# Immortalqx/pi-slam-fusion

Measured on AMD Instinct MI355X. Metric: keyframes/sec fused (4000x3000 -> 256^2 tiles, 5-band), higher is better.
Workload: dtype f32; 1 GPU; cfg-2/cfg-A: 4000x3000 BGR8 keyframes, serpentine sortie, Map2D.Scale=1, 5-band Laplacian, CV_32FC3 (ForceFloat=1) pyramids, frames resident in HBM; frames_per_rank=2646, sortie_frames_before_timing=20, lookahead=48, rendered_rank0=2666, culled_tiles_rank0=490117

## Files before the change

include/pifusion.h:

```cpp
#ifndef PIFUSION_H
#define PIFUSION_H
#include <stddef.h>
#include <stdint.h>

#ifdef __cplusplus
extern "C" {
#endif

#define PF_ELE_PIXELS 256

enum { PF_TYPE_NONE = 0, PF_TYPE_CPU = 1, PF_TYPE_GPU = 2, PF_TYPE_MULTIBAND = 3, PF_TYPE_RENDER = 4 };

enum { PF_8UC1 = 0, PF_8UC3 = 16, PF_8UC4 = 24, PF_16SC3 = 19, PF_32FC1 = 5, PF_32FC3 = 21 };

typedef struct pf_image {
    int         rows, cols, type;
    const void* data;
    size_t      step;
} pf_image;

typedef struct pf_options {
    int    band_number;
    int    force_float;
    int    high_quality_show;
    int    weight_type;
    int    bg_color;
    double resolution;
    double scale;
    int    device;
    int    shard_rank;
    int    shard_count;
    int    shard_block;
    int    max_queue;
    int    fused;
    int    lookahead;
} pf_options;

typedef struct pf_map pf_map;

void    pf_default_options(pf_options* o);
int     pf_options_set(pf_options* o, const char* key, const char* value);
pf_map* pf_create(int type, int thread, const pf_options* opt);
void    pf_destroy(pf_map* m);
const char* pf_last_error(void);

int     pf_prepare(pf_map* m, const double plane[7], const double cam[6],
                   int n, const pf_image* imgs, const double* poses7);
int     pf_feed(pf_map* m, const pf_image* img, const double pose[7]);
int     pf_feed_device(pf_map* m, const pf_image* img, const double pose[7]);
long    pf_debug_read_last_frame(pf_map* m, void* out, size_t cap);
int     pf_debug_phase_stamps(unsigned long long* out, int cap_blocks);
int     pf_debug_select_counts(unsigned long long* out, int reset);
unsigned pf_queue_size(pf_map* m);
int     pf_sync(pf_map* m);
int     pf_save(pf_map* m, const char* filename);
int     pf_save_tiff(pf_map* m, const char* filename, int quality, int force_bigtiff);
int     pf_save_tiff_masked(pf_map* m, const char* filename, int quality, int force_bigtiff);
int     pf_write_image(const char* filename, const uint8_t* bgr, int rows, int cols);
int     pf_tiff_write_bgr(const char* filename, const uint8_t* bgr, int rows, int cols, size_t step, int quality, int bg,
                          const double model_transform[16], int force_bigtiff);
int     pf_tiff_write_device(const char* filename, const void* dev_bgr, int rows, int cols, size_t step, int quality, int bg,
                             const double model_transform[16], int force_bigtiff, void* hip_stream);
int     pf_tiff_write_bgr_masked(const char* filename, const uint8_t* bgr, int rows, int cols, size_t step,
                                 const uint8_t* mask, size_t mask_step, int quality, int bg,
                                 const double model_transform[16], int force_bigtiff);
int     pf_tiff_write_device_masked(const char* filename, const void* dev_bgr, int rows, int cols, size_t step,
                                    const void* dev_mask, size_t mask_step, int quality, int bg,
                                    const double model_transform[16], int force_bigtiff, void* hip_stream);
int     pf_jpeg_encode_bgr(const uint8_t* bgr, int rows, int cols, size_t step, int quality, uint8_t* out, size_t cap, size_t* len);
int     pf_jpeg_encode_device(const void* dev_bgr, int rows, int cols, size_t step, int quality, uint8_t* out, size_t cap, size_t* len, void* hip_stream);
int     pf_image_info(const char* filename, int* rows, int* cols);
int     pf_read_image(const char* filename, uint8_t* bgr, int rows, int cols);
int     pf_jpeg_info(const uint8_t* data, size_t len, int* rows, int* cols, int* components);
int     pf_jpeg_decode_bgr(const uint8_t* data, size_t len, uint8_t* bgr, int rows, int cols);
int     pf_jpeg_decode_device(const uint8_t* data, size_t len, void* dev_bgr, int rows, int cols, void* hip_stream);
void    pf_debug_jpeg_huffman(pf_map* m, long long out[3]);
int     pf_feed_jpeg(pf_map* m, const uint8_t* data, size_t len, const double pose[7]);
int     pf_feed_jpeg_batch(pf_map* m, int n, const uint8_t* const* data, const size_t* len, const double* poses7, int threads, int* results);
int     pf_save_to_memory(pf_map* m, uint8_t* bgr, int* rows, int* cols, int* tile_x0, int* tile_y0);
int     pf_save_to_memory_mask(pf_map* m, uint8_t* bgr, uint8_t* mask, int* rows, int* cols, int* tile_x0, int* tile_y0);

int     pf_num_levels(pf_map* m);
int     pf_pyramid_type(pf_map* m);
int     pf_grid(pf_map* m, int dims[4], double geo[6]);
int     pf_tile_count(pf_map* m);
int     pf_tile_coords(pf_map* m, int* xy, int cap);
int     pf_get_tile_level(pf_map* m, int ix, int iy, int level, void* lap, float* w);
int     pf_get_tile_bgra(pf_map* m, int ix, int iy, uint8_t* bgra256);
int     pf_blend_tile_raw(pf_map* m, int ix, int iy, void* out);
int     pf_blend_tile(pf_map* m, int ix, int iy, uint8_t* bgr256);
int     pf_blend_changed(pf_map* m, int* xy, uint8_t* bgr, int cap);
int     pf_blend_tiles(pf_map* m, const int* xy, int n, uint8_t* bgr);
int     pf_blend_tiles_jpeg(pf_map* m, const int* xy, int n, int quality, uint8_t* out, size_t cap, size_t* offsets);
int     pf_blend_tiles_level(pf_map* m, const int* xy, int n, int level, uint8_t* bgr, void* raw);
int     pf_blend_changed_level(pf_map* m, int level, int* xy, uint8_t* bgr, int cap);
int     pf_save_to_memory_level(pf_map* m, int level, uint8_t* bgr, int* rows, int* cols, int* tile_x0, int* tile_y0);
void*   pf_host_alloc(size_t bytes);
void    pf_host_free(void* p);
int     pf_format_map_update(const double plane[7], const double gps_origin[3], double min_x, double min_y, double ele_size,
                             int x, int y, char* out, int cap);
int     pf_map_update_command(pf_map* m, int ix, int iy, const double gps_origin[3], char* out, int cap);
void    pf_lnglat_from_distance(double lng1, double lat1, double dx, double dy, double* lng2, double* lat2);
int     pf_normalize_using_weight_map(const float* weight, float* src3, size_t npix);
int     pf_mul_weight_map(const float* weight, float* src3, size_t npix);

// ... 64 lines not shown
```

pi-slam-fusion_amd/csrc/c_api.cpp:

```cpp
#include "dist.hpp"
#include "jpeg_device.hpp"
#include <cstdlib>
#include <cmath>
#include <cstdio>
#include <cstring>
#include <algorithm>
#include <vector>
#include <mutex>
#include <new>

using pf::FusionMap;

struct pf_map {
    FusionMap impl;
    pf::JpegDevice jpeg;
    pf_map(int t, bool th, const pf_options& o) : impl(t, th, o) {}
    ~pf_map() { if (impl.ok() && impl.use_device()) impl.sync(); }
};

static std::mutex g_jpeg_mu;
static pf::JpegDevice* shared_jpeg(int device = 0)
{
    static pf::JpegDevice* d[64] = {};
    if (device < 0 || device >= 64) device = 0;
// ... 9 lines not shown
    o->resolution = 0; o->scale = 1; o->device = -1; o->shard_rank = 0; o->shard_count = 1; o->shard_block = 8;
    o->max_queue = 20; o->fused = 1; o->lookahead = 48;
}

int pf_options_set(pf_options* o, const char* key, const char* value)
{
    if (!o || !key || !value) return 0;
    const double v = std::atof(value);
    if (!std::strcmp(key, "MultiBandMap2DCPU.BandNumber")) o->band_number = (int)v;
    else if (!std::strcmp(key, "MultiBandMap2DCPU.ForceFloat")) o->force_float = (int)v;
    else if (!std::strcmp(key, "MultiBandMap2DCPU.HighQualityShow")) o->high_quality_show = (int)v;
    else if (!std::strcmp(key, "Map2D.WeightType")) o->weight_type = (int)v;
    else if (!std::strcmp(key, "Result.BackGroundColor")) o->bg_color = (int)v;
    else if (!std::strcmp(key, "Map2D.Resolution")) o->resolution = v;
    else if (!std::strcmp(key, "Map2D.Scale")) o->scale = v;
    else if (!std::strcmp(key, "Device")) o->device = (int)v;
    else if (!std::strcmp(key, "Shard.Rank")) o->shard_rank = (int)v;
    else if (!std::strcmp(key, "Shard.Count")) o->shard_count = (int)v;
    else if (!std::strcmp(key, "Shard.Block")) o->shard_block = (int)v;
    else if (!std::strcmp(key, "Map2D.MaxQueue")) o->max_queue = (int)v;
    else if (!std::strcmp(key, "Fused")) o->fused = (int)v;
    else if (!std::strcmp(key, "Lookahead")) o->lookahead = (int)v;
    else return 0;
    return 1;
}

pf_map* pf_create(int type, int thread, const pf_options* opt)
{
    if (type == PF_TYPE_NONE || type == PF_TYPE_RENDER) return nullptr;
    pf_options o;
    if (opt) o = *opt; else pf_default_options(&o);
    pf_map* m = new (std::nothrow) pf_map(type, thread != 0, o);
    if (m && !m->impl.ok()) { delete m; return nullptr; }
    return m;
}

void pf_destroy(pf_map* m) { delete m; }
const char* pf_last_error(void) { return pf::last_error(); }

int pf_prepare(pf_map* m, const double plane[7], const double cam[6], int n, const pf_image* imgs, const double* poses7)
{ return m && m->impl.prepare(plane, cam, n, imgs, poses7); }

int pf_feed(pf_map* m, const pf_image* img, const double pose[7]) { return m && m->impl.feed(img, pose, false); }
int pf_feed_device(pf_map* m, const pf_image* img, const double pose[7]) { return m && m->impl.feed(img, pose, true); }
int pf_debug_phase_stamps(unsigned long long* out, int cap_blocks) { return pf::read_phase_stamps(out, cap_blocks); }
void pf_debug_form_counts(long long out[8]) { if (out) pf::read_form_counts(out); }
long long pf_debug_compact_launches(void) { return pf::read_compact_launches(); }
int pf_debug_render_log(pf_map* m, long long* out, int cap) { return m ? m->impl.render_log(out, cap) : 0; }
void pf_set_cull(pf_map* m, int on) { if (m) m->impl.set_cull(on != 0); }
long long pf_debug_culled_cells(pf_map* m) { return m ? m->impl.culled_cells() : 0; }
double pf_debug_level0_exact_px(pf_map* m) { return m ? m->impl.level0_exact_px() : 0; }
long long pf_debug_culled_tiles(pf_map* m) { return m ? m->impl.culled_tiles() : 0; }
int pf_debug_select_counts(unsigned long long* out, int reset) { return out ? pf::read_select_counts(out, reset) : 0; }
long pf_debug_read_last_frame(pf_map* m, void* out, size_t cap) { return m ? m->impl.read_back_last_frame(out, cap) : -1; }
unsigned pf_queue_size(pf_map* m) { return m ? m->impl.queue_size() : 0; }
int pf_sync(pf_map* m) { return m && m->impl.sync(); }
int pf_save(pf_map* m, const char* filename) { return m && filename && m->impl.save(filename); }
int pf_save_tiff(pf_map* m, const char* filename, int quality, int force_bigtiff) { return m && filename && m->impl.save_tiff(filename, quality, force_bigtiff != 0); }
int pf_save_tiff_masked(pf_map* m, const char* filename, int quality, int force_bigtiff) { return m && filename && m->impl.save_tiff_masked(filename, quality, force_bigtiff != 0); }
int pf_jpeg_info(const uint8_t* data, size_t len, int* rows, int* cols, int* components) { return pf::jpeg_info(data, len, rows, cols, components); }
int pf_jpeg_decode_bgr(const uint8_t* data, size_t len, uint8_t* bgr, int rows, int cols)
{ return rows > 0 && cols > 0 && pf::jpeg_decode_bgr(data, len, bgr, rows, cols, (size_t)cols * 3); }
int pf_jpeg_decode_device(const uint8_t* data, size_t len, void* dev_bgr, int rows, int cols, void* hip_stream)
{
    std::lock_guard<std::mutex> l(g_jpeg_mu);
    if (rows <= 0 || cols <= 0 || !dev_bgr) return 0;
    hipPointerAttribute_t at{};
    if (hipPointerGetAttributes(&at, dev_bgr) != hipSuccess || at.type != hipMemoryTypeDevice) { (void)hipGetLastError(); pf::set_error("pf_jpeg_decode_device: destination is not device memory"); return 0; }
    int prev = 0;
    (void)hipGetDevice(&prev);
    if (at.device != prev && hipSetDevice(at.device) != hipSuccess) { pf::set_error("pf_jpeg_decode_device: hipSetDevice failed"); return 0; }
    const int ok = shared_jpeg(at.device)->decode_to(data, len, (uint8_t*)dev_bgr, rows, cols, hip_stream);
    if (at.device != prev) (void)hipSetDevice(prev);
    return ok;
}
static pf::JpegEncoder* shared_jpeg_encoder(int device)
{
    static pf::JpegEncoder* e[64] = {};
    if (device < 0 || device >= 64) device = 0;
    if (!e[device]) e[device] = new pf::JpegEncoder();
    return e[device];
}
int pf_jpeg_encode_device(const void* dev_bgr, int rows, int cols, size_t step, int quality, uint8_t* out, size_t cap, size_t* len, void* hip_stream)
{
    std::lock_guard<std::mutex> l(g_jpeg_mu);
    if (!dev_bgr || !len || rows <= 0 || cols <= 0) { pf::set_error("pf_jpeg_encode_device: no image, no length or a size that is not positive"); return 0; }
    if (!pf::jpeg_size_ok("pf_jpeg_encode_device", rows, cols)) return 0;
    if (step == 0) step = (size_t)cols * 3;
    if (step < (size_t)cols * 3) { pf::set_error("pf_jpeg_encode_device: step is smaller than a row"); return 0; }
    if (!out) { *len = pf::jenc::stream_bound(rows, cols); return 1; }
    hipPointerAttribute_t at{};
    if (hipPointerGetAttributes(&at, dev_bgr) != hipSuccess || at.type != hipMemoryTypeDevice) { (void)hipGetLastError(); pf::set_error("pf_jpeg_encode_device: the image is not in device memory"); return 0; }
    int prev = 0;
    (void)hipGetDevice(&prev);
    if (at.device != prev && hipSetDevice(at.device) != hipSuccess) { pf::set_error("pf_jpeg_encode_device: hipSetDevice failed"); return 0; }
    pf::JpegEncoder* e = shared_jpeg_encoder(at.device);
    size_t off[2] = { 0, 0 };
    int ok = e->encode(dev_bgr, 1, nullptr, 0, rows, cols, step, quality, off, hip_stream);
    if (ok) {
        *len = off[1];
        if (off[1] > cap) {
            pf::set_error("pf_jpeg_encode_device: the stream has " + std::to_string(off[1]) + " bytes, the buffer " + std::to_string(cap));
            (void)hipStreamSynchronize((hipStream_t)hip_stream);
            ok = 0;
        } else ok = e->fetch(out, hip_stream);
    }
// ... 308 lines not shown
```

pi-slam-fusion_amd/csrc/kernels.hip:

```cpp
#include "kernels.hpp"
#include "warp_index.hpp"
#include "env.hpp"
#include <climits>
#include <cmath>
#include <cstdlib>
#include <type_traits>

#ifndef PF_EXPERIMENTS
#define PF_EXPERIMENTS 0
#endif
#ifndef PF_ROWTAB
#define PF_ROWTAB 0
#endif
#ifndef PF_HYBRID_W
#define PF_HYBRID_W 0
#endif

namespace pf {

constexpr bool kExp = PF_EXPERIMENTS != 0;

__device__ __forceinline__ double clamp_int_range(double v)
{
    v = (v < (double)INT_MAX) ? v : (double)INT_MAX;
// ... 753 lines not shown
        }
        u.w = 0.f;
        U[p][lx] = u;
    }
    lds_barrier();
#pragma unroll
    for (int it = 0; it < ND; it++) {
        const uint64_t ent = ents[it];
        if (!ent) continue;
        const int idx = tid + it * LNT, ly = idx >> 6, lx = idx & 63;
        const int y = y0 + ly, x = x0 + lx;
        const Px gpx = A[ly + 4][lx + 4];
        if (!(gpx.w >= dwv[it])) continue;
        const uint64_t slot = ent & ~(uint64_t)1;
        const int loc = (y & (ts - 1)) * ts + (x & (ts - 1));
        const int sy = y >> 1;
        int syn = sy + 1; if (syn >= nrows) syn = nrows - 1;
        int syp = sy - 1; if (syp < 0) syp = nrows > 1 ? 1 : 0;
        const Hx u1 = U[sy - by0][lx], u2 = U[syn - by0][lx];
        T out[3];
        if (y & 1) {
#pragma unroll
            for (int k = 0; k < 3; k++) out[k] = sat_sub(gpx.c[k], cast_up((u1.c[k] + u2.c[k]) * 4));
        } else {
            const Hx u0 = U[syp - by0][lx];
#pragma unroll
            for (int k = 0; k < 3; k++) out[k] = sat_sub(gpx.c[k], cast_up(u0.c[k] + u1.c[k] * 6 + u2.c[k]));
        }
        T PF_GLOBAL* dl = (T PF_GLOBAL*)(slot + lay.lap_off) + loc * 3;
        dl[0] = out[0]; dl[1] = out[1]; dl[2] = out[2];
        ((float PF_GLOBAL*)(slot + lay.w_off))[loc] = gpx.w;
    }
    if (st + 1 < LS) {
        lds_barrier();
        Px keep;
        const bool mv = tid < 7 * LAW;
        if (mv) keep = (&A[0][0])[LBH * LAW + tid];
        lds_barrier();
        if (mv) (&A[0][0])[tid] = keep;
    }
    }
}

__device__ __forceinline__ void phase_stamp(unsigned long long* st, int slot)
{
    if (st) {
        unsigned long long t;
        asm volatile("s_memtime %0\n\ts_waitcnt lgkmcnt(0)" : "=s"(t) :: "memory");
        if (threadIdx.x == 0) st[slot] = t;
    }
}

__device__ unsigned long long g_select_seen[kMaxLevels], g_select_won[kMaxLevels];

constexpr int kPatchBytes = 81920 - 44928;

template <bool F32, int LBH, int LNT, bool STAMP = false, int ILP = 2, bool PATCH = false, bool WA = false, class LO = LevelOffsets, class GA = LevelArgs>
__device__ __forceinline__ void level3_block(const bool FROM_WARP, const LO& lay, const GA& g, const FusedWarp& wa,
                                             const uint8_t* __restrict__ src, const PxT<F32>* __restrict__ gw_in,
                                             PxT<F32>* __restrict__ gw_out, const uint64_t* __restrict__ table_generic, const int b,
                                             unsigned long long* stamps = nullptr, const uint64_t* tab0 = nullptr)
{
    const uint64_t PF_GLOBAL* __restrict__ table = (const uint64_t PF_GLOBAL*)table_generic;
    if (STAMP) phase_stamp(stamps, 0);
    struct StampExit { unsigned long long* st; __device__ StampExit(unsigned long long* p) : st(p) {} __device__ ~StampExit() { asm volatile("s_waitcnt vmcnt(0)" ::: "memory"); phase_stamp(st, 5); } };
    struct NoExit { __device__ NoExit(unsigned long long*) {} };
    typename std::conditional<STAMP, StampExit, NoExit>::type at_exit(stamps);
    (void)at_exit;
    using T = typename Pix<F32>::T; using WT = typename Pix<F32>::WT;
    using Px = PxT<F32>;
    constexpr int LAH = LBH + 7, LQH = LBH / 2 + 2;
    static_assert(LNT >= 32 * (LBH / 2), "one thread per 2x2 output quad (threads beyond that help in stages A and B only)");
    struct Bx { T c[F32 ? 3 : 4]; };
    constexpr int kPitch = LBH == 24 ? LAW : 2 * LAWH;
    __shared__ Px A[LAH][kPitch];
    constexpr int kTail = PATCH ? kPatchBytes : (int)(sizeof(Bx) * LQH * LQW);
    static_assert(kTail >= (int)(sizeof(Bx) * LQH * LQW), "Bt must fit");
    __shared__ __attribute__((aligned(16))) unsigned char tail[kTail];
    Bx (*Bt)[LQW] = reinterpret_cast<Bx (*)[LQW]>(tail);
    auto Aat = [&](int r, int c) -> Px& { return A[r][(c & 1) * LAWH + (c >> 1)]; };
    static_assert(LBH != 32 || PATCH || sizeof(A) + sizeof(tail) <= (F32 ? 42 : 32) * 1280, "LDS budget (64x32 blocks)");
    static_assert(LBH != 24 || sizeof(A) + sizeof(tail) <= 32 * 1280, "LDS budget (64x24 blocks: four workgroups per CU for both pyramid types)");
    static_assert(LBH != 32 || !PATCH || sizeof(A) + sizeof(tail) <= 64 * 1280, "LDS budget (64x32 blocks with a source patch: two per CU)");
    static_assert(LBH != 64 || sizeof(A) + sizeof(tail) <= (F32 ? 128 : 64) * 1280, "LDS budget (64x64 blocks of 1024 threads: int16 two per CU, fp32 one)");

    int bx, by; block_xy(g, b, bx, by);
    const int x0 = g.cx0 + bx * LBW, y0 = g.cy0 + by * LBH;
    const int ax0 = x0 - 4, ay0 = y0 - 4;
    const int nrows = g.rows >> 1, ncols = g.cols >> 1;
    const int bx0 = (x0 >> 1) - 1, by0 = (y0 >> 1) - 1;
    const int tid = threadIdx.x;
    const int sh = 8 - g.level, ts = kElePixels >> g.level;
    if (kExp && (g.ablate & 512) && !FROM_WARP) __builtin_amdgcn_s_setprio(2);

    const int qx = tid & 31, qy = tid >> 5;
    const int dx0 = x0 + 2 * qx, dy0 = y0 + 2 * qy;
    uint64_t ent = 0;
    if (tid < 32 * (LBH / 2) && dx0 < g.cols && dy0 < g.rows) {
        const int ti = (dy0 >> sh) * g.tiles_x + (dx0 >> sh);
        if (tab0) ent = ((const uint64_t PF_GLOBAL*)tab0)[ti];
        else ent = table[ti];
        if (sh >= 3) { if (cell_culled(ent, dx0, dy0, ts, sh)) ent = 0; }
        else {
            bool all = true;
#pragma unroll
            for (int k = 0; k < 4; k++) all = all && cell_culled(ent, dx0 + (k & 1), dy0 + (k >> 1), ts, sh);
            if (all) ent = 0;
        }
        ent &= ~kEntCells;
    }

    if (kExp && FROM_WARP && (g.ablate & 1024) && tid >= LNT / 2) __builtin_amdgcn_s_setprio(1);
    if (kExp && FROM_WARP && (g.ablate & 2048) && tid < LNT / 2) __builtin_amdgcn_s_setprio(1);
    if (FROM_WARP) {
        const bool inner = ax0 >= 0 && ax0 + LAW <= g.cols && ay0 >= 0 && ay0 + LAH <= g.rows;
        constexpr int RS = LNT / LAW;
        const int r0 = tid / LAW, c = tid - r0 * LAW;
        const bool near101 = g.rows >= 8 && g.cols >= 8;
        auto col_of = [&](int cc) {
            int x = ax0 + cc;
            if (!inner) x = near101 ? border_reflect101_near(x, g.cols) : border_reflect101(x, g.cols);
            return x;
        };
        auto row_of = [&](int r) {
            int y = ay0 + r;
            if (!inner) y = near101 ? border_reflect101_near(y, g.rows) : border_reflect101(y, g.rows);
            return y;
        };
// ... 317 lines not shown
            auto emit = [&](int e) {
                const int p = 2 * pp + e, Y = by0 + p;
                if (Y < 0 || Y >= nrows) return;
                Px o;
                {
                    const us2 v01 = h01[2 * e + 2] * (us2)6 + (h01[2 * e + 1] + h01[2 * e + 3]) * (us2)4 + h01[2 * e] + h01[2 * e + 4];
                    const us2 v2p = h2p[2 * e + 2] * (us2)6 + (h2p[2 * e + 1] + h2p[2 * e + 3]) * (us2)4 + h2p[2 * e] + h2p[2 * e + 4];
                    const us2 o01 = (v01 + (us2)128) >> (us2)8, o2p = (v2p + (us2)128) >> (us2)8;
                    o.c[0] = (short)o01.x; o.c[1] = (short)o01.y; o.c[2] = (short)o2p.x;
                }
                {
                    const float r0 = hw[2 * e], r1 = hw[2 * e + 1], r2 = hw[2 * e + 2], r3 = hw[2 * e + 3], r4 = hw[2 * e + 4];
                    if (X < vec_w) {
                        float a = r0 + r4;
                        const float bb = (r1 + r3) + r2;
                        a = a + (r2 + r2);
                        o.w = (a + bb * 4.f) * (1.f / 256);
                    } else
                        o.w = (r2 * 6 + (r1 + r3) * 4 + r0 + r4) * (1.f / 256);
                }
                o.pad = 0;
                {
                    Bx ob; ob.c[0] = o.c[0]; ob.c[1] = o.c[1]; ob.c[2] = o.c[2]; ob.c[3] = 0;
                    Bt[p][q] = ob;
                }
                if (p >= 1 && p < LQH - 1 && q >= 1 && q < LQW - 1) {
                    if (kExp && (g.ablate & 4096)) {
                        typedef uint32_t u2g __attribute__((ext_vector_type(2)));
                        u2g v; __builtin_memcpy(&v, &o, 8);
                        if (g.write_next) ((u2g*)gw_out)[(long)Y * ncols + X] = v;
                    } else
                    if (g.write_next) gw_out[(long)Y * ncols + X] = o;
                    if (g.top_select) select_store<F32>(lay.top_lap_off, lay.top_w_off, g.level + 1, table, g.tiles_x, X, Y, o.c, o.w);
                }
            };
#pragma unroll
            for (int j = 0; j < 7; j++) {
                const PxP* ev = reinterpret_cast<const PxP*>(&A[4 * pp + j][q]); const PxP* od = reinterpret_cast<const PxP*>(&A[4 * pp + j][LAWH + q]);
                const PxP a0 = ev[0], a1 = od[0], a2 = ev[1], a3 = od[1], a4 = ev[2];
                h01[j] = a2.c01 * (us2)6 + (a1.c01 + a3.c01) * (us2)4 + a0.c01 + a4.c01;
                h2p[j] = a2.c2p * (us2)6 + (a1.c2p + a3.c2p) * (us2)4 + a0.c2p + a4.c2p;
                hw[j] = a2.w * 6 + (a1.w + a3.w) * 4 + a0.w + a4.w;
                asm volatile("" : "+v"(h01[j]), "+v"(h2p[j]), "+v"(hw[j]) :: "memory");
                if (j == 4) emit(0);
                if (j == 6) emit(1);
            }
        }
    }
    if (STAMP) phase_stamp(stamps, 3);
    lds_barrier();
    if (STAMP) phase_stamp(stamps, 4);
    if (kExp && (g.ablate & 4)) return;

    if (!ent) return;
    int ry = dy0;
    asm volatile("" : "+v"(ry));
    ry -= y0;
    const Px g00 = A[ry + 4][qx + 2], g01 = A[ry + 4][LAWH + qx + 2];
    const Px g10 = A[ry + 5][qx + 2], g11 = A[ry + 5][LAWH + qx + 2];
    const bool in01 = dx0 + 1 < g.cols, in10 = dy0 + 1 < g.rows;
    const bool s00 = g00.w >= dwv[0][0], s01 = in01 && g01.w >= dwv[0][1];
    const bool s10 = in10 && g10.w >= dwv[1][0], s11 = in10 && in01 && g11.w >= dwv[1][1];
#ifdef PF_COUNT_WINS
    if constexpr (STAMP) {
        atomicAdd(&g_select_seen[g.level], (unsigned long long)(1 + (int)in01 + (int)in10 + (int)(in10 && in01)));
        atomicAdd(&g_select_won[g.level], (unsigned long long)((int)s00 + (int)s01 + (int)s10 + (int)s11));
    }
#endif
    if (!(s00 || s01 || s10 || s11)) return;
    const int sy = dy0 >> 1, sx = dx0 >> 1;
    int syn = sy + 1; if (syn >= nrows) syn = nrows - 1;
    int syp = sy - 1; if (syp < 0) syp = nrows > 1 ? 1 : 0;
    const bool one = ncols == 1, le = sx == 0, re = sx == ncols - 1;
    const bool edge = le || re;
    const int j = qx + 1;
    const int ja = (le && !F32) ? (one ? j : j + 1) : j - 1, jc = (re && !F32) ? j : j + 1;
    const int rows3[3] = { syp - by0, sy - by0, syn - by0 };
    T PF_GLOBAL* dl = (T PF_GLOBAL*)(slot + lay.lap_off) + loc0 * 3;
    float PF_GLOBAL* dw = (float PF_GLOBAL*)(slot + lay.w_off) + loc0;
    if constexpr (F32) {
        if (__builtin_amdgcn_ballot_w64(edge) == 0) {
            f2 heL[3], hoL[3]; float he2[3], ho2[3];
#pragma unroll
            for (int r = 0; r < 3; r++) {
                const float* pa = Bt[rows3[r]][j - 1].c; const float* pb = Bt[rows3[r]][j].c; const float* pc = Bt[rows3[r]][j + 1].c;
                const f2 aL = { pa[0], pa[1] }, bL = { pb[0], pb[1] }, cL = { pc[0], pc[1] };
                const float a2 = pa[2], b2 = pb[2], c2 = pc[2];
                heL[r] = aL + bL * 6.f + cL; hoL[r] = (bL + cL) * 4.f;
                he2[r] = a2 + b2 * 6 + c2;   ho2[r] = (b2 + c2) * 4;
            }
            const f2 g00L = { g00.c[0], g00.c[1] }, g01L = { g01.c[0], g01.c[1] }, g10L = { g10.c[0], g10.c[1] }, g11L = { g11.c[0], g11.c[1] };
            const f2 o00L = g00L - (heL[0] + heL[1] * 6.f + heL[2]) * (1.f / 64);
            const f2 o01L = g01L - (hoL[0] + hoL[1] * 6.f + hoL[2]) * (1.f / 64);
            const f2 o10L = g10L - ((heL[1] + heL[2]) * 4.f) * (1.f / 64);
            const f2 o11L = g11L - ((hoL[1] + hoL[2]) * 4.f) * (1.f / 64);
            const float o00c = g00.c[2] - (he2[0] + he2[1] * 6 + he2[2]) * (1.f / 64);
            const float o01c = g01.c[2] - (ho2[0] + ho2[1] * 6 + ho2[2]) * (1.f / 64);
            const float o10c = g10.c[2] - ((he2[1] + he2[2]) * 4) * (1.f / 64);
            const float o11c = g11.c[2] - ((ho2[1] + ho2[2]) * 4) * (1.f / 64);
            auto st3 = [&](T PF_GLOBAL* p, float a, float b, float c2) { PF_STORE(p, a); PF_STORE(p + 1, b); PF_STORE(p + 2, c2); };
            if (s00) { st3(dl, o00L.x, o00L.y, o00c); PF_STORE_W(&dw[0], g00.w); }
            if (s01) { st3(dl + 3, o01L.x, o01L.y, o01c); PF_STORE_W(&dw[1], g01.w); }
            if (s10) { st3(dl + 3 * ts, o10L.x, o10L.y, o10c); PF_STORE_W(&dw[ts], g10.w); }
            if (s11) { st3(dl + 3 * ts + 3, o11L.x, o11L.y, o11c); PF_STORE_W(&dw[ts + 1], g11.w); }
            return;
        }
    }
    if constexpr (!F32) {
        ss2 he01[3], ho01[3], he2p[3], ho2p[3];
#pragma unroll
        for (int r = 0; r < 3; r++) {
            const BxP a = *reinterpret_cast<const BxP*>(&Bt[rows3[r]][ja]), bq = *reinterpret_cast<const BxP*>(&Bt[rows3[r]][j]),
                      c = *reinterpret_cast<const BxP*>(&Bt[rows3[r]][jc]);
            he01[r] = a.c01 + bq.c01 * (ss2)6 + c.c01; ho01[r] = (bq.c01 + c.c01) * (ss2)4;
            he2p[r] = a.c2p + bq.c2p * (ss2)6 + c.c2p; ho2p[r] = (bq.c2p + c.c2p) * (ss2)4;
        }
        auto up_e = [](ss2 u0, ss2 u1, ss2 u2) { return (u0 + u1 * (ss2)6 + u2 + (ss2)32) >> (ss2)6; };
        auto up_o = [](ss2 u1, ss2 u2) { return ((u1 + u2) * (ss2)4 + (ss2)32) >> (ss2)6; };
        auto px2 = [](const Px& q, ss2& c01, ss2& c2p) { const PxP& v = reinterpret_cast<const PxP&>(q); c01 = (ss2)v.c01; c2p = (ss2)v.c2p; };
        ss2 a01, a2p;
        auto st3p = [&](T PF_GLOBAL* p, ss2 c01, ss2 c2p) { PF_STORE(p, c01.x); PF_STORE(p + 1, c01.y); PF_STORE(p + 2, c2p.x); };
        if (s00) { px2(g00, a01, a2p); st3p(dl, a01 - up_e(he01[0], he01[1], he01[2]), a2p - up_e(he2p[0], he2p[1], he2p[2])); PF_STORE_W(&dw[0], g00.w); }
        if (s01) { px2(g01, a01, a2p); st3p(dl + 3, a01 - up_e(ho01[0], ho01[1], ho01[2]), a2p - up_e(ho2p[0], ho2p[1], ho2p[2])); PF_STORE_W(&dw[1], g01.w); }
        if (s10) { px2(g10, a01, a2p); st3p(dl + 3 * ts, a01 - up_o(he01[1], he01[2]), a2p - up_o(he2p[1], he2p[2])); PF_STORE_W(&dw[ts], g10.w); }
        if (s11) { px2(g11, a01, a2p); st3p(dl + 3 * ts + 3, a01 - up_o(ho01[1], ho01[2]), a2p - up_o(ho2p[1], ho2p[2])); PF_STORE_W(&dw[ts + 1], g11.w); }
        return;
    }
    WT he[3][3], ho[3][3];
#pragma unroll
    for (int r = 0; r < 3; r++) {
        const Bx a = Bt[rows3[r]][ja], bq = Bt[rows3[r]][j], c = Bt[rows3[r]][jc];
#pragma unroll
        for (int k = 0; k < 3; k++) {
            if (F32 && edge) {
                he[r][k] = up_h_val<WT, true>((WT)a.c[k], (WT)bq.c[k], (WT)c.c[k], false, le, re, one);
                ho[r][k] = up_h_val<WT, true>((WT)a.c[k], (WT)bq.c[k], (WT)c.c[k], true, le, re, one);
            } else {
                he[r][k] = up_h_val<WT, false>((WT)a.c[k], (WT)bq.c[k], (WT)c.c[k], false, false, false, false);
                ho[r][k] = up_h_val<WT, false>((WT)a.c[k], (WT)bq.c[k], (WT)c.c[k], true, false, false, false);
            }
        }
    }
    T o00[3], o01[3], o10[3], o11[3];
#pragma unroll
    for (int k = 0; k < 3; k++) {
        o00[k] = sat_sub(g00.c[k], cast_up(he[0][k] + he[1][k] * 6 + he[2][k]));
        o01[k] = sat_sub(g01.c[k], cast_up(ho[0][k] + ho[1][k] * 6 + ho[2][k]));
        o10[k] = sat_sub(g10.c[k], cast_up((he[1][k] + he[2][k]) * 4));
        o11[k] = sat_sub(g11.c[k], cast_up((ho[1][k] + ho[2][k]) * 4));
    }
    auto st3g = [&](T PF_GLOBAL* p, const T* v) { PF_STORE(p, v[0]); PF_STORE(p + 1, v[1]); PF_STORE(p + 2, v[2]); };
    if (s00) { st3g(dl, o00); PF_STORE_W(&dw[0], g00.w); }
    if (s01) { st3g(dl + 3, o01); PF_STORE_W(&dw[1], g01.w); }
    if (s10) { st3g(dl + 3 * ts, o10); PF_STORE_W(&dw[ts], g10.w); }
    if (s11) { st3g(dl + 3 * ts + 3, o11); PF_STORE_W(&dw[ts + 1], g11.w); }
}

__device__ __forceinline__ int xcd_order(int b, int nblk)
{
    const int per = nblk >> 3;
    return (per > 0 && b < per * 8) ? (b & 7) * per + (b >> 3) : b;
}

__device__ __forceinline__ int xcd_chunks(int b, int nblk, int C)
{
    const int full = (nblk / (8 * C)) * (8 * C);
    if (b >= full) return b;
    const int k = b >> 3;
    return ((k / C) * 8 + (b & 7)) * C + k % C;
}

template <bool F32, bool FROM_WARP, int LBH, int LNT>
__global__ __launch_bounds__(LNT, 4) void k_level3(LevelOffsets lay, LevelArgs g, FusedWarp wa, const uint8_t* __restrict__ src,
                                                 const PxT<F32>* __restrict__ gw_in, PxT<F32>* __restrict__ gw_out,
                                                 const uint64_t* __restrict__ table)
{
    level3_block<F32, LBH, LNT>(FROM_WARP, lay, g, wa, src, gw_in, gw_out, table, xcd_order(blockIdx.x, g.nbx * g.nby));
}

struct LevelJob {
    LevelArgs    g;
    int first;
    int from_warp;
    int nrect;
    int bits_off;
    LevelOffsets lay;
    const void*  gw_in;
    void*        gw_out;
    const uint64_t* table;
    BlockRect rect[kMaxRectsUpper];
};
static_assert(sizeof(LevelArgs) == 64 && offsetof(LevelJob, first) == 64 && offsetof(LevelJob, lay) == 80 && sizeof(LevelJob) == 152, "LevelJob layout (k_levels loads its first 20 dwords by hand)");
#define PF_CONST __attribute__((address_space(4)))
typedef uint32_t su16 __attribute__((ext_vector_type(16)));
typedef uint32_t su8 __attribute__((ext_vector_type(8)));
typedef uint32_t su4 __attribute__((ext_vector_type(4)));
typedef uint32_t su2 __attribute__((ext_vector_type(2)));
template <int N>
__device__ __forceinline__ void load_words(const char PF_CONST* p, uint32_t (&w)[N])
{
    static_assert(N % 4 == 0, "whole 16-byte groups");
    int i = 0;
#pragma unroll
    for (; i + 16 <= N; i += 16) { const su16 v = *(const su16 PF_CONST*)(p + 4 * i); for (int k = 0; k < 16; k++) w[i + k] = v[k]; }
#pragma unroll
    for (; i + 4 <= N; i += 4) { const su4 v = *(const su4 PF_CONST*)(p + 4 * i); for (int k = 0; k < 4; k++) w[i + k] = v[k]; }
}

// ... 485 lines not shown
    }
    if (ilp_env == 0 && !wplane && !lay.f32) {
        if (wa) g_form_counts[0]++;
        PF_GO(false, 32, 512, false, 0, false, true);
        return;
    }
    if (ilp_env == 2 || ilp_env == 3) {
        if (wa) g_form_counts[wplane ? 1 : 0]++;
        if (wplane) {
            if (lay.f32) { if (ilp_env == 3) PF_GO(true, 32, 512, false, 3, false, false); else PF_GO(true, 32, 512, false, 2, false, false); }
            else         { if (ilp_env == 3) PF_GO(false, 32, 512, false, 3, false, false); else PF_GO(false, 32, 512, false, 2, false, false); }
        } else {
            if (lay.f32) { if (ilp_env == 3) PF_GO(true, 32, 512, false, 3, false, true); else PF_GO(true, 32, 512, false, 2, false, true); }
            else         { if (ilp_env == 3) PF_GO(false, 32, 512, false, 3, false, true); else PF_GO(false, 32, 512, false, 2, false, true); }
        }
        return;
    }
#undef PF_GO
#endif
    if (wa) g_form_counts[wplane ? 1 : 0]++;
    if (wplane) {
        if (lay.f32) hipLaunchKernelGGL((k_levels<true, 32, 512, false, 3, false, false>), dim3(nblocks), dim3(512), 0, s, batch, w, src, st);
        else         hipLaunchKernelGGL((k_levels<false, 32, 512, false, 2, false, false>), dim3(nblocks), dim3(512), 0, s, batch, w, src, st);
    } else {
        if (lay.f32) hipLaunchKernelGGL((k_levels<true, 32, 512, false, 0, false, true>), dim3(nblocks), dim3(512), 0, s, batch, w, src, st);
        else         hipLaunchKernelGGL((k_levels<false, 32, 512, false, 2, false, true>), dim3(nblocks), dim3(512), 0, s, batch, w, src, st);
    }
}

int level_block_rows(bool f32)
{
    (void)f32;
#if PF_EXPERIMENTS
    static const bool b64 = getenv("PF_BLOCK64") != nullptr, b28 = getenv("PF_BLOCK28") != nullptr, b24 = getenv("PF_BLOCK24") != nullptr;
    return b64 ? 64 : (b28 ? 28 : (b24 ? 24 : 32));
#else
    return 32;
#endif
}

int read_select_counts(unsigned long long* out, int reset)
{
    unsigned long long seen[kMaxLevels], won[kMaxLevels];
    if (hipMemcpyFromSymbol(seen, HIP_SYMBOL(g_select_seen), sizeof seen) != hipSuccess) return 0;
    if (hipMemcpyFromSymbol(won, HIP_SYMBOL(g_select_won), sizeof won) != hipSuccess) return 0;
    for (int i = 0; i < kMaxLevels; i++) { out[2 * i] = seen[i]; out[2 * i + 1] = won[i]; }
    if (reset) {
        unsigned long long z[kMaxLevels] = {};
        (void)hipMemcpyToSymbol(HIP_SYMBOL(g_select_seen), z, sizeof z); (void)hipMemcpyToSymbol(HIP_SYMBOL(g_select_won), z, sizeof z);
    }
    return kMaxLevels;
}

int read_phase_stamps(unsigned long long* out, int cap_blocks)
{
    if (!g_stamp_buf || !g_stamp_blocks) return 0;
    const int n = g_stamp_blocks < cap_blocks ? g_stamp_blocks : cap_blocks;
    if (out && hipMemcpy(out, g_stamp_buf, (size_t)n * 64, hipMemcpyDeviceToHost) != hipSuccess) return 0;
    return n;
}

__host__ __device__ inline void strip_dims(int nlev, int level, int dx, int dy, int& w, int& h)
{
    const int ts = kElePixels >> level, b = 1 << (nlev - 1 - level);
    w = dx == 0 ? ts : b; h = dy == 0 ? ts : b;
}

size_t halo_bytes(const TileLayout& lay, int dx, int dy)
{
    size_t n = 0;
    for (int i = 0; i < lay.nlev; i++) { int w, h; strip_dims(lay.nlev, i, dx, dy, w, h); n += (size_t)w * h; }
    return n * 3 * (lay.f32 ? 4 : 2);
}

#if PF_EXPERIMENTS
template <bool F32>
__global__ __launch_bounds__(256) void k_blend_gather(TileLayout lay, int level, int border, const BlendSrc* __restrict__ srcs,
                                                       char* __restrict__ dst, size_t dst_stride)
{
    using T = typename Pix<F32>::T;
    const int ts = kElePixels >> level, side = ts + 2 * border;
    const int px = blockIdx.x * 64 + (threadIdx.x & 63), py = blockIdx.y * 4 + (threadIdx.x >> 6);
    if (px >= side || py >= side) return;
    const int z = blockIdx.z;
    int rx, sx, ry, sy;
    if (px < border) { rx = 0; sx = ts - border + px; } else if (px < border + ts) { rx = 1; sx = px - border; } else { rx = 2; sx = px - border - ts; }
    if (py < border) { ry = 0; sy = ts - border + py; } else if (py < border + ts) { ry = 1; sy = py - border; } else { ry = 2; sy = py - border - ts; }
    const BlendSrc bs = srcs[z * 9 + ry * 3 + rx];
    T* d = reinterpret_cast<T*>(dst + z * dst_stride) + ((long)py * side + px) * 3;
    const T* s;
    if (!bs.is_strip) {
        s = reinterpret_cast<const T*>(reinterpret_cast<const char*>(bs.base) + lay.lap_off[level]) + ((long)sy * ts + sx) * 3;
    } else {
        const int dx = rx - 1, dy = ry - 1;
        long off = 0;
        for (int i = 0; i < level; i++) { int w, h; strip_dims(lay.nlev, i, dx, dy, w, h); off += (long)w * h; }
        int w, h; strip_dims(lay.nlev, level, dx, dy, w, h);
        const int lx = (rx == 0) ? sx - (ts - border) : sx, ly = (ry == 0) ? sy - (ts - border) : sy;
        s = reinterpret_cast<const T*>(bs.base) + (off + (long)ly * w + lx) * 3;
    }
    d[0] = s[0]; d[1] = s[1]; d[2] = s[2];
}

void launch_blend_gather(hipStream_t s, const TileLayout& lay, int level, int border, const BlendSrc* srcs,
                         void* dst, size_t dst_stride_bytes, int batch)
{
// ... 195 lines not shown
```

pi-slam-fusion_amd/csrc/kernels.hpp:

```cpp
#pragma once
#include "plan_limits.hpp"
#include <hip/hip_runtime.h>
#include <cstdint>
#include <cstddef>

namespace pf {

struct TileLayout {
    int      nlev;
    int      f32;
    uint32_t lap_off[kMaxLevels];
    uint32_t w_off[kMaxLevels];
    uint32_t slot_bytes;
};

TileLayout make_layout(int band_num, bool f32);

struct WarpArgs {
    double M[9];
    int    srows, scols;
    long   sstep;
    int    crows, ccols;
    int    y_off, x_off;
    int    wrows, wcols;
// ... 1 lines not shown
    int    weight_type;
    const float* wmap;
    int    src_cn;
};

struct BlendSrc {
    const void* base;
    int         is_strip;
};

struct BlendJob {
    uint64_t src[9];
    uint32_t strip_mask;
    int      border;
    int      out;
    int      pad_;
};
static_assert(sizeof(BlendJob) == 88, "BlendJob is copied to LDS by words");

enum KernelId { K_WARP = 0, K_PYRDOWN_IMG, K_PYRDOWN_W, K_LAP_SELECT, K_BLEND_GATHER, K_COLLAPSE,
                K_BLEND_FINISH, K_MOSAIC_GATHER, K_SAVE_FINISH, K_LEVEL0, K_LEVEL, K_SINGLE, K_BLEND_FUSED, K_SAVE_FUSED, K_BLEND_LEVEL, K_SAVE_LEVEL, K_COUNT };
const char* kernel_name(int id);

void launch_warp(hipStream_t s, bool f32, const uint8_t* src, const WarpArgs& a, void* g0, float* w0);

void launch_pyrdown(hipStream_t s, int type, const void* src, int srows, int scols, void* dst,
                    int y0, int y1, int x0, int x1);

void launch_lap_select(hipStream_t s, const TileLayout& lay, int level, const void* g_i, const void* g_up,
                       const float* w_i, int rows, int cols, const uint64_t* tile_table, int tiles_x,
                       int ty0, int ty1, int tx0, int tx1);

size_t level_px_bytes(bool f32);
void launch_level(hipStream_t s, const TileLayout& lay, int level, int rows, int cols, int cx0, int cy0, int cx1, int cy1,
                  int tiles_x, bool top_select, bool write_next, const WarpArgs* wa, const uint8_t* src,
                  const void* gw_in, void* gw_out, const uint64_t* table, int shape = 3);

struct LevelLaunch {
    int level, rows, cols;
    int cx0, cy0, cx1, cy1;
    int tiles_x;
    bool top_select, write_next, from_warp;
    const void* gw_in; void* gw_out;
    const uint64_t* table;
    const uint64_t* table_args; int table_n;
    int nrect; BlockRect rect[kMaxRects];
    const uint32_t* need_bits = nullptr; int need_n = 0;
};
void launch_levels(hipStream_t s, const TileLayout& lay, const LevelLaunch* jobs, int njobs, const WarpArgs* wa, const uint8_t* src);
int  read_phase_stamps(unsigned long long* out, int cap_blocks);
void read_form_counts(long long out[8]);
long long read_compact_launches();
int  read_select_counts(unsigned long long* out, int reset);
int  level0_need_reach(const TileLayout& lay, int table_n, int nrect0);
int  level_block_rows(bool f32);

void launch_blend_fused(hipStream_t s, const TileLayout& lay, const BlendJob* jobs_dev, int n, void* raw_out, uint8_t* bgr_out);
void launch_save_fused(hipStream_t s, const TileLayout& lay, const uint64_t* table_dev, int wx, int wy, int bg, uint8_t* bgr_out);
void launch_blend_level(hipStream_t s, const TileLayout& lay, int level, const BlendJob* jobs_dev, int n, void* raw_out, uint8_t* bgr_out);
void launch_save_level(hipStream_t s, const TileLayout& lay, int level, const uint64_t* table_dev, int wx, int wy, int bg, uint8_t* bgr_out);

void launch_blend_gather(hipStream_t s, const TileLayout& lay, int level, int border, const BlendSrc* srcs,
                         void* dst, size_t dst_stride_bytes, int batch);
void launch_collapse(hipStream_t s, bool f32, void* dst, size_t dst_stride_bytes, const void* src,
                     size_t src_stride_bytes, int rows, int cols, int batch);
void launch_blend_finish(hipStream_t s, const TileLayout& lay, const void* lvl0, size_t stride_bytes, int border,
                         const BlendSrc* srcs, void* raw_out, uint8_t* bgr_out, int batch, const int* out_idx = nullptr);

void launch_mosaic_gather(hipStream_t s, const TileLayout& lay, int level, const uint64_t* table, int wx, int wy, void* dst);
void launch_save_finish(hipStream_t s, const TileLayout& lay, const void* lvl0, const uint64_t* table, int wx, int wy,
                        int bg, uint8_t* bgr);

size_t halo_bytes(const TileLayout& lay, int dx, int dy);
void launch_halo_pack(hipStream_t s, const TileLayout& lay, const void* slot, int dx, int dy, void* out);
struct StripDesc { const void* slot; int dx, dy; size_t out_off; };
void launch_halo_pack_batch(hipStream_t s, const TileLayout& lay, const StripDesc* descs_dev, int n, void* out);

void launch_weight8(hipStream_t s, uint8_t* w, int rows, int cols, int weight_type);
void launch_weight32(hipStream_t s, float* w, int rows, int cols, int weight_type);
void launch_single(hipStream_t s, const uint8_t* src, const uint8_t* w8, const WarpArgs& a, const uint64_t* table, int tiles_x);

}
```

Baseline: 26860 keyframes/s.

## Stage Laplacian select stores through LDS for wide coalesced writes

When every lane in a wave wins the select and all lanes target the same aligned tile slot, the Laplacian and weight outputs go into shared-memory scratch rows and are written back as 16-byte (or 8-byte) vector stores instead of scattered per-channel stores. Other waves use a per-row store helper that merges paired stores where both pixels win. The aim is to cut the number of global store instructions and improve coalescing in the select kernel. The cost is extra wave ballots and readfirstlane checks, LDS traffic, and reuse of rows of the A tile as scratch. A debug counter for wave store categories is also added.

Result: slower. 26280 keyframes/s (-2.2%).

```diff
diff --git a/include/pifusion.h b/include/pifusion.h
--- a/include/pifusion.h
+++ b/include/pifusion.h
@@ -51,6 +51,7 @@
 long    pf_debug_read_last_frame(pf_map* m, void* out, size_t cap);
 int     pf_debug_phase_stamps(unsigned long long* out, int cap_blocks);
 int     pf_debug_select_counts(unsigned long long* out, int reset);
+int     pf_debug_select_waves(unsigned long long* out, int reset);
 unsigned pf_queue_size(pf_map* m);
 int     pf_sync(pf_map* m);
 int     pf_save(pf_map* m, const char* filename);
diff --git a/pi-slam-fusion_amd/csrc/c_api.cpp b/pi-slam-fusion_amd/csrc/c_api.cpp
--- a/pi-slam-fusion_amd/csrc/c_api.cpp
+++ b/pi-slam-fusion_amd/csrc/c_api.cpp
@@ -85,6 +85,7 @@
 double pf_debug_level0_exact_px(pf_map* m) { return m ? m->impl.level0_exact_px() : 0; }
 long long pf_debug_culled_tiles(pf_map* m) { return m ? m->impl.culled_tiles() : 0; }
 int pf_debug_select_counts(unsigned long long* out, int reset) { return out ? pf::read_select_counts(out, reset) : 0; }
+int pf_debug_select_waves(unsigned long long* out, int reset) { return out ? pf::read_select_waves(out, reset) : 0; }
 long pf_debug_read_last_frame(pf_map* m, void* out, size_t cap) { return m ? m->impl.read_back_last_frame(out, cap) : -1; }
 unsigned pf_queue_size(pf_map* m) { return m ? m->impl.queue_size() : 0; }
 int pf_sync(pf_map* m) { return m && m->impl.sync(); }
diff --git a/pi-slam-fusion_amd/csrc/kernels.hip b/pi-slam-fusion_amd/csrc/kernels.hip
--- a/pi-slam-fusion_amd/csrc/kernels.hip
+++ b/pi-slam-fusion_amd/csrc/kernels.hip
@@ -829,6 +829,9 @@
 }
 
 __device__ unsigned long long g_select_seen[kMaxLevels], g_select_won[kMaxLevels];
+__device__ unsigned long long g_select_waves[kMaxLevels * 4];
+
+constexpr bool kWideSelect = true;
 
 constexpr int kPatchBytes = 81920 - 44928;
 
@@ -850,7 +853,7 @@
     static_assert(LNT >= 32 * (LBH / 2), "one thread per 2x2 output quad (threads beyond that help in stages A and B only)");
     struct Bx { T c[F32 ? 3 : 4]; };
     constexpr int kPitch = LBH == 24 ? LAW : 2 * LAWH;
-    __shared__ Px A[LAH][kPitch];
+    __shared__ __attribute__((aligned(16))) Px A[LAH][kPitch];
     constexpr int kTail = PATCH ? kPatchBytes : (int)(sizeof(Bx) * LQH * LQW);
     static_assert(kTail >= (int)(sizeof(Bx) * LQH * LQW), "Bt must fit");
     __shared__ __attribute__((aligned(16))) unsigned char tail[kTail];
@@ -1274,7 +1277,8 @@
     if (STAMP) phase_stamp(stamps, 4);
     if (kExp && (g.ablate & 4)) return;
 
-    if (!ent) return;
+    const bool has = ent != 0;
+    if (__builtin_amdgcn_ballot_w64(has) == 0) return;
     int ry = dy0;
     asm volatile("" : "+v"(ry));
     ry -= y0;
@@ -1283,6 +1287,28 @@
     const bool in01 = dx0 + 1 < g.cols, in10 = dy0 + 1 < g.rows;
     const bool s00 = g00.w >= dwv[0][0], s01 = in01 && g01.w >= dwv[0][1];
     const bool s10 = in10 && g10.w >= dwv[1][0], s11 = in10 && in01 && g11.w >= dwv[1][1];
+    const int sy = dy0 >> 1, sx = dx0 >> 1;
+    const bool one = ncols == 1, le = sx == 0, re = sx == ncols - 1;
+    const bool edge = le || re;
+    T PF_GLOBAL* dl = (T PF_GLOBAL*)(slot + lay.lap_off) + loc0 * 3;
+    float PF_GLOBAL* dw = (float PF_GLOBAL*)(slot + lay.w_off) + loc0;
+    bool wide = false;
+    {
+        bool off_grid = false;
+        const bool allwin = __builtin_amdgcn_ballot_w64(has && s00 && s01 && s10 && s11) == ~0ull;
+        if (kWideSelect && allwin && !(kExp && (g.ablate & 8192))) {
+            const uint32_t slo = (uint32_t)slot, shi = (uint32_t)(slot >> 32);
+            const bool same = slo == (uint32_t)__builtin_amdgcn_readfirstlane((int)slo) && shi == (uint32_t)__builtin_amdgcn_readfirstlane((int)shi);
+            const uint32_t al = (uint32_t)__builtin_amdgcn_readfirstlane((int)(uint32_t)(uint64_t)dl), aw = (uint32_t)__builtin_amdgcn_readfirstlane((int)(uint32_t)(uint64_t)dw);
+            const bool one_tile = __builtin_amdgcn_ballot_w64(same && !(F32 && edge)) == ~0ull;
+            wide = one_tile && ((al & (F32 ? 15u : 7u)) | (aw & 15u)) == 0;
+            off_grid = one_tile && !wide;
+        }
+        if constexpr (STAMP) {
+            if ((tid & 63) == 0) atomicAdd(&g_select_waves[g.level * 4 + (wide ? 2 : (off_grid ? 3 : (allwin ? 1 : 0)))], 1ull);
+        }
+    }
+    if (!has) return;
 #ifdef PF_COUNT_WINS
     if constexpr (STAMP) {
         atomicAdd(&g_select_seen[g.level], (unsigned long long)(1 + (int)in01 + (int)in10 + (int)(in10 && in01)));
@@ -1290,16 +1316,71 @@
     }
 #endif
     if (!(s00 || s01 || s10 || s11)) return;
-    const int sy = dy0 >> 1, sx = dx0 >> 1;
     int syn = sy + 1; if (syn >= nrows) syn = nrows - 1;
     int syp = sy - 1; if (syp < 0) syp = nrows > 1 ? 1 : 0;
-    const bool one = ncols == 1, le = sx == 0, re = sx == ncols - 1;
-    const bool edge = le || re;
     const int j = qx + 1;
     const int ja = (le && !F32) ? (one ? j : j + 1) : j - 1, jc = (re && !F32) ? j : j + 1;
     const int rows3[3] = { syp - by0, sy - by0, syn - by0 };
-    T PF_GLOBAL* dl = (T PF_GLOBAL*)(slot + lay.lap_off) + loc0 * 3;
-    float PF_GLOBAL* dw = (float PF_GLOBAL*)(slot + lay.w_off) + loc0;
+    constexpr int ND = F32 ? 6 : 3;
+    using DW = typename std::conditional<F32, float, uint32_t>::type;
+    typedef uint32_t u32m __attribute__((may_alias));
+    typedef uint32_t u2m __attribute__((ext_vector_type(2), may_alias));
+    typedef uint32_t u4m __attribute__((ext_vector_type(4), may_alias));
+    auto narrow_row = [&](T PF_GLOBAL* p, float PF_GLOBAL* pw, bool sa, bool sb, const DW (&v)[ND], float wa_, float wb_) {
+        if (sa && sb) {
+            if constexpr (F32) {
+#pragma unroll
+                for (int k = 0; k < 6; k++) PF_STORE(p + k, v[k]);
+            } else {
+                u32m PF_GLOBAL* q = (u32m PF_GLOBAL*)p;
+                PF_STORE(q, v[0]); PF_STORE(q + 1, v[1]); PF_STORE(q + 2, v[2]);
+            }
+            f2 wv; wv.x = wa_; wv.y = wb_;
+            PF_STORE_W((f2 PF_GLOBAL*)pw, wv);
+        } else if (sa) {
+            if constexpr (F32) { PF_STORE(p, v[0]); PF_STORE(p + 1, v[1]); PF_STORE(p + 2, v[2]); }
+            else { PF_STORE(p, (T)(v[0] & 0xffff)); PF_STORE(p + 1, (T)(v[0] >> 16)); PF_STORE(p + 2, (T)(v[1] & 0xffff)); }
+            PF_STORE_W(pw, wa_);
+        } else if (sb) {
+            if constexpr (F32) { PF_STORE(p + 3, v[3]); PF_STORE(p + 4, v[4]); PF_STORE(p + 5, v[5]); }
+            else { PF_STORE(p + 3, (T)(v[1] >> 16)); PF_STORE(p + 4, (T)(v[2] & 0xffff)); PF_STORE(p + 5, (T)(v[2] >> 16)); }
+            PF_STORE_W(pw + 1, wb_);
+        }
+    };
+    auto wide_store = [&](const DW (&top)[ND], const DW (&bot)[ND]) {
+        constexpr int SP = F32 ? 1024 : 640, WO = F32 ? 768 : 384, CB = F32 ? 16 : 8;
+        constexpr int RP = (int)(sizeof(Px) * kPitch);
+        static_assert(WO == 64 * 3 * (int)sizeof(T) && WO + 256 <= SP && SP <= RP && SP % 16 == 0 && (4 * RP) % 16 == 0, "scratch rows fit the wave's rows of A");
+        static_assert(LBH % 4 == 0 && LBH + 4 <= LAH, "a wave with quads (tid < 32 * LBH / 2) owns four whole rows of A");
+        const int lq = tid & 63;
+        char* S = reinterpret_cast<char*>(&A[0][0]) + (4 * (tid >> 6) + 4) * RP;
+        char* mine = S + (lq >> 5) * (2 * SP);
+        u32m* t = reinterpret_cast<u32m*>(mine + qx * (ND * 4)); u32m* bq = reinterpret_cast<u32m*>(mine + SP + qx * (ND * 4));
+#pragma unroll
+        for (int k = 0; k < ND; k++) {
+            if constexpr (F32) { t[k] = __float_as_uint(top[k]); bq[k] = __float_as_uint(bot[k]); }
+            else { t[k] = top[k]; bq[k] = bot[k]; }
+        }
+        { u2m v; v.x = __float_as_uint(g00.w); v.y = __float_as_uint(g01.w); *reinterpret_cast<u2m*>(mine + WO + 8 * qx) = v; }
+        { u2m v; v.x = __float_as_uint(g10.w); v.y = __float_as_uint(g11.w); *reinterpret_cast<u2m*>(mine + SP + WO + 8 * qx) = v; }
+        asm volatile("s_waitcnt lgkmcnt(0)" ::: "memory");
+        auto first64 = [](uint64_t v) { return (uint64_t)(uint32_t)__builtin_amdgcn_readfirstlane((int)(uint32_t)v) | (uint64_t)(uint32_t)__builtin_amdgcn_readfirstlane((int)(uint32_t)(v >> 32)) << 32; };
+        const uint64_t bl = first64((uint64_t)dl), bw = first64((uint64_t)dw);
+        const uint32_t lrow = (uint32_t)ts * 3 * (uint32_t)sizeof(T), wrow = (uint32_t)ts * 4;
+#pragma unroll
+        for (int k = 0; k < 3; k++) {
+            const int c = k * 64 + lq, row = c / 48, col = c - row * 48;
+            const char* sp = S + row * SP + col * CB;
+            const uint64_t gp = bl + (uint64_t)((uint32_t)row * lrow + (uint32_t)(col * CB));
+            if constexpr (F32) PF_STORE((u4m PF_GLOBAL*)gp, *reinterpret_cast<const u4m*>(sp));
+            else               PF_STORE((u2m PF_GLOBAL*)gp, *reinterpret_cast<const u2m*>(sp));
+        }
+        {
+            const int row = lq >> 4, col = lq & 15;
+            PF_STORE_W((u4m PF_GLOBAL*)(bw + (uint64_t)((uint32_t)row * wrow + (uint32_t)(col * 16))), *reinterpret_cast<const u4m*>(S + row * SP + WO + col * 16));
+        }
+    };
+    DW top[ND], bot[ND];
     if constexpr (F32) {
         if (__builtin_amdgcn_ballot_w64(edge) == 0) {
             f2 heL[3], hoL[3]; float he2[3], ho2[3];
@@ -1316,15 +1397,13 @@
             const f2 o01L = g01L - (hoL[0] + hoL[1] * 6.f + hoL[2]) * (1.f / 64);
             const f2 o10L = g10L - ((heL[1] + heL[2]) * 4.f) * (1.f / 64);
             const f2 o11L = g11L - ((hoL[1] + hoL[2]) * 4.f) * (1.f / 64);
-            const float o00c = g00.c[2] - (he2[0] + he2[1] * 6 + he2[2]) * (1.f / 64);
-            const float o01c = g01.c[2] - (ho2[0] + ho2[1] * 6 + ho2[2]) * (1.f / 64);
-            const float o10c = g10.c[2] - ((he2[1] + he2[2]) * 4) * (1.f / 64);
-            const float o11c = g11.c[2] - ((ho2[1] + ho2[2]) * 4) * (1.f / 64);
-            auto st3 = [&](T PF_GLOBAL* p, float a, float b, float c2) { PF_STORE(p, a); PF_STORE(p + 1, b); PF_STORE(p + 2, c2); };
-            if (s00) { st3(dl, o00L.x, o00L.y, o00c); PF_STORE_W(&dw[0], g00.w); }
-            if (s01) { st3(dl + 3, o01L.x, o01L.y, o01c); PF_STORE_W(&dw[1], g01.w); }
-            if (s10) { st3(dl + 3 * ts, o10L.x, o10L.y, o10c); PF_STORE_W(&dw[ts], g10.w); }
-            if (s11) { st3(dl + 3 * ts + 3, o11L.x, o11L.y, o11c); PF_STORE_W(&dw[ts + 1], g11.w); }
+            top[0] = o00L.x; top[1] = o00L.y; top[2] = g00.c[2] - (he2[0] + he2[1] * 6 + he2[2]) * (1.f / 64);
+            top[3] = o01L.x; top[4] = o01L.y; top[5] = g01.c[2] - (ho2[0] + ho2[1] * 6 + ho2[2]) * (1.f / 64);
+            bot[0] = o10L.x; bot[1] = o10L.y; bot[2] = g10.c[2] - ((he2[1] + he2[2]) * 4) * (1.f / 64);
+            bot[3] = o11L.x; bot[4] = o11L.y; bot[5] = g11.c[2] - ((ho2[1] + ho2[2]) * 4) * (1.f / 64);
+            if (wide) { wide_store(top, bot); return; }
+            narrow_row(dl, dw, s00, s01, top, g00.w, g01.w);
+            narrow_row(dl + 3 * ts, dw + ts, s10, s11, bot, g10.w, g11.w);
             return;
         }
     }
@@ -1340,42 +1419,46 @@
         auto up_e = [](ss2 u0, ss2 u1, ss2 u2) { return (u0 + u1 * (ss2)6 + u2 + (ss2)32) >> (ss2)6; };
         auto up_o = [](ss2 u1, ss2 u2) { return ((u1 + u2) * (ss2)4 + (ss2)32) >> (ss2)6; };
         auto px2 = [](const Px& q, ss2& c01, ss2& c2p) { const PxP& v = reinterpret_cast<const PxP&>(q); c01 = (ss2)v.c01; c2p = (ss2)v.c2p; };
-        ss2 a01, a2p;
-        auto st3p = [&](T PF_GLOBAL* p, ss2 c01, ss2 c2p) { PF_STORE(p, c01.x); PF_STORE(p + 1, c01.y); PF_STORE(p + 2, c2p.x); };
-        if (s00) { px2(g00, a01, a2p); st3p(dl, a01 - up_e(he01[0], he01[1], he01[2]), a2p - up_e(he2p[0], he2p[1], he2p[2])); PF_STORE_W(&dw[0], g00.w); }
-        if (s01) { px2(g01, a01, a2p); st3p(dl + 3, a01 - up_e(ho01[0], ho01[1], ho01[2]), a2p - up_e(ho2p[0], ho2p[1], ho2p[2])); PF_STORE_W(&dw[1], g01.w); }
-        if (s10) { px2(g10, a01, a2p); st3p(dl + 3 * ts, a01 - up_o(he01[1], he01[2]), a2p - up_o(he2p[1], he2p[2])); PF_STORE_W(&dw[ts], g10.w); }
-        if (s11) { px2(g11, a01, a2p); st3p(dl + 3 * ts + 3, a01 - up_o(ho01[1], ho01[2]), a2p - up_o(ho2p[1], ho2p[2])); PF_STORE_W(&dw[ts + 1], g11.w); }
+        auto pack = [](DW (&v)[ND], ss2 a01, ss2 a2p, ss2 b01, ss2 b2p) {
+            uint32_t ua, ub; __builtin_memcpy(&ua, &a01, 4); __builtin_memcpy(&ub, &b01, 4);
+            v[0] = ua; v[1] = (uint32_t)(uint16_t)a2p.x | ub << 16; v[2] = ub >> 16 | (uint32_t)(uint16_t)b2p.x << 16;
+        };
+        ss2 a01, a2p, b01, b2p;
+        px2(g00, a01, a2p); px2(g01, b01, b2p);
+        pack(top, a01 - up_e(he01[0], he01[1], he01[2]), a2p - up_e(he2p[0], he2p[1], he2p[2]), b01 - up_e(ho01[0], ho01[1], ho01[2]), b2p - up_e(ho2p[0], ho2p[1], ho2p[2]));
+        px2(g10, a01, a2p); px2(g11, b01, b2p);
+        pack(bot, a01 - up_o(he01[1], he01[2]), a2p - up_o(he2p[1], he2p[2]), b01 - up_o(ho01[1], ho01[2]), b2p - up_o(ho2p[1], ho2p[2]));
+        if (wide) { wide_store(top, bot); return; }
+        narrow_row(dl, dw, s00, s01, top, g00.w, g01.w);
+        narrow_row(dl + 3 * ts, dw + ts, s10, s11, bot, g10.w, g11.w);
         return;
     }
-    WT he[3][3], ho[3][3];
-#pragma unroll
-    for (int r = 0; r < 3; r++) {
-        const Bx a = Bt[rows3[r]][ja], bq = Bt[rows3[r]][j], c = Bt[rows3[r]][jc];
+    if constexpr (F32) {
+        WT he[3][3], ho[3][3];
+#pragma unroll
+        for (int r = 0; r < 3; r++) {
+            const Bx a = Bt[rows3[r]][ja], bq = Bt[rows3[r]][j], c = Bt[rows3[r]][jc];
+#pragma unroll
+            for (int k = 0; k < 3; k++) {
+                if (edge) {
+                    he[r][k] = up_h_val<WT, true>((WT)a.c[k], (WT)bq.c[k], (WT)c.c[k], false, le, re, one);
+                    ho[r][k] = up_h_val<WT, true>((WT)a.c[k], (WT)bq.c[k], (WT)c.c[k], true, le, re, one);
+                } else {
+                    he[r][k] = up_h_val<WT, false>((WT)a.c[k], (WT)bq.c[k], (WT)c.c[k], false, false, false, false);
+                    ho[r][k] = up_h_val<WT, false>((WT)a.c[k], (WT)bq.c[k], (WT)c.c[k], true, false, false, false);
+                }
+            }
+        }
 #pragma unroll
         for (int k = 0; k < 3; k++) {
-            if (F32 && edge) {
-                he[r][k] = up_h_val<WT, true>((WT)a.c[k], (WT)bq.c[k], (WT)c.c[k], false, le, re, one);
-                ho[r][k] = up_h_val<WT, true>((WT)a.c[k], (WT)bq.c[k], (WT)c.c[k], true, le, re, one);
-            } else {
-                he[r][k] = up_h_val<WT, false>((WT)a.c[k], (WT)bq.c[k], (WT)c.c[k], false, false, false, false);
-                ho[r][k] = up_h_val<WT, false>((WT)a.c[k], (WT)bq.c[k], (WT)c.c[k], true, false, false, false);
-            }
-        }
-    }
-    T o00[3], o01[3], o10[3], o11[3];
-#pragma unroll
-    for (int k = 0; k < 3; k++) {
-        o00[k] = sat_sub(g00.c[k], cast_up(he[0][k] + he[1][k] * 6 + he[2][k]));
-        o01[k] = sat_sub(g01.c[k], cast_up(ho[0][k] + ho[1][k] * 6 + ho[2][k]));
-        o10[k] = sat_sub(g10.c[k], cast_up((he[1][k] + he[2][k]) * 4));
-        o11[k] = sat_sub(g11.c[k], cast_up((ho[1][k] + ho[2][k]) * 4));
-    }
-    auto st3g = [&](T PF_GLOBAL* p, const T* v) { PF_STORE(p, v[0]); PF_STORE(p + 1, v[1]); PF_STORE(p + 2, v[2]); };
-    if (s00) { st3g(dl, o00); PF_STORE_W(&dw[0], g00.w); }
-    if (s01) { st3g(dl + 3, o01); PF_STORE_W(&dw[1], g01.w); }
-    if (s10) { st3g(dl + 3 * ts, o10); PF_STORE_W(&dw[ts], g10.w); }
-    if (s11) { st3g(dl + 3 * ts + 3, o11); PF_STORE_W(&dw[ts + 1], g11.w); }
+            top[k] = sat_sub(g00.c[k], cast_up(he[0][k] + he[1][k] * 6 + he[2][k]));
+            top[3 + k] = sat_sub(g01.c[k], cast_up(ho[0][k] + ho[1][k] * 6 + ho[2][k]));
+            bot[k] = sat_sub(g10.c[k], cast_up((he[1][k] + he[2][k]) * 4));
+            bot[3 + k] = sat_sub(g11.c[k], cast_up((ho[1][k] + ho[2][k]) * 4));
+        }
+        narrow_row(dl, dw, s00, s01, top, g00.w, g01.w);
+        narrow_row(dl + 3 * ts, dw + ts, s10, s11, bot, g10.w, g11.w);
+    }
 }
 
 __device__ __forceinline__ int xcd_order(int b, int nblk)
@@ -1967,6 +2050,15 @@
     return kMaxLevels;
 }
 
+int read_select_waves(unsigned long long* out, int reset)
+{
+    unsigned long long v[kMaxLevels * 4];
+    if (hipMemcpyFromSymbol(v, HIP_SYMBOL(g_select_waves), sizeof v) != hipSuccess) return 0;
+    for (int i = 0; i < kMaxLevels * 4; i++) out[i] = v[i];
+    if (reset) { unsigned long long z[kMaxLevels * 4] = {}; (void)hipMemcpyToSymbol(HIP_SYMBOL(g_select_waves), z, sizeof z); }
+    return kMaxLevels;
+}
+
 int read_phase_stamps(unsigned long long* out, int cap_blocks)
 {
     if (!g_stamp_buf || !g_stamp_blocks) return 0;
diff --git a/pi-slam-fusion_amd/csrc/kernels.hpp b/pi-slam-fusion_amd/csrc/kernels.hpp
--- a/pi-slam-fusion_amd/csrc/kernels.hpp
+++ b/pi-slam-fusion_amd/csrc/kernels.hpp
@@ -77,6 +77,7 @@
 void read_form_counts(long long out[8]);
 long long read_compact_launches();
 int  read_select_counts(unsigned long long* out, int reset);
+int  read_select_waves(unsigned long long* out, int reset);
 int  level0_need_reach(const TileLayout& lay, int table_n, int nrect0);
 int  level_block_rows(bool f32);
 
```
